# RupertLuo/Valley

Hardware: AMD Instinct MI355X
Metric: frames/sec ViT-L/14 encode + prefill tokens/sec (13B) (higher is better)
Workload: dtype bf16

## Files before the change

valley_amd/csrc/attention.hip:

```cpp
#include <cstdlib>
#include "common.hpp"
#include "../../include/valley_hip.h"

namespace {

constexpr float LOG2E = 1.4426950408889634f;
constexpr float NEG_BIG = -1.0e30f;

#ifndef VLY_DECODE_MERGE_FENCE
#define VLY_DECODE_MERGE_FENCE 0
#endif
#ifndef VLY_VIT_PRIO
#define VLY_VIT_PRIO 0
#endif
#ifndef VLY_VIT_STAGGER
#define VLY_VIT_STAGGER 0
#endif
#ifndef VLY_VIT_TIMING
#define VLY_VIT_TIMING 0
#endif
#ifndef VLY_VIT_STAGE2
#define VLY_VIT_STAGE2 1
#endif
#ifndef VLY_VIT_ROT
// ... 222 lines not shown
#pragma unroll
            for (int kk = 0; kk < 2; ++kk) {
                const bf16x8 kf = *(const bf16x8*)(sK + (t * 16 + l15) * 128 + (((kk * 4 + g) ^ (l15 & 7)) << 4));
                acc = mfma16(kf, qf[kk], acc);
            }
#if VLY_VIT_FOLD
            s[t] = acc;
#else
            s[t] = acc * sc;
#endif
            if ((t & 3) == 3) asm volatile("" ::: "memory");
        }
#if VLY_VIT_PRIO
        __builtin_amdgcn_s_setprio(0);
#endif
#pragma unroll
        for (int r = 0; r < 4; ++r)
            if (g != 0 || r != 0) s[VNT - 1][r] = NEG_BIG;
#if VLY_VIT_TIMING
        asm volatile("" : "+v"(s[VNT - 1][0]));
        VLY_VSTAMP();
#endif

        float m = NEG_BIG;
        float l = 0.f;
#if VLY_VIT_FOLD
#pragma unroll
        for (int t = 0; t < VNT; ++t) {
            m = __builtin_fmaxf(__builtin_fmaxf(m, s[t][0]), s[t][1]);
            m = __builtin_fmaxf(__builtin_fmaxf(m, s[t][2]), s[t][3]);
        }
        m = rows4_max(m);
        {
            const float nm = -m * sc;
            float l2 = 0.f;
#pragma unroll
            for (int t = 0; t < VNT; ++t) {
                const float p0 = sm_exp2(__builtin_fmaf(s[t][0], sc, nm)), p1 = sm_exp2(__builtin_fmaf(s[t][1], sc, nm));
                const float p2 = sm_exp2(__builtin_fmaf(s[t][2], sc, nm)), p3 = sm_exp2(__builtin_fmaf(s[t][3], sc, nm));
                s[t] = f32x4{p0, p1, p2, p3};
                l += p0 + p1;
                l2 += p2 + p3;
            }
            l += l2;
        }
#else
#pragma unroll
        for (int t = 0; t < VNT; ++t)
#pragma unroll
            for (int r = 0; r < 4; ++r) m = fmaxf(m, s[t][r]);
        m = rows4_max(m);
#pragma unroll
        for (int t = 0; t < VNT; ++t)
#pragma unroll
            for (int r = 0; r < 4; ++r) {
                const float p = sm_exp2(s[t][r] - m);
                s[t][r] = p;
                l += p;
            }
#endif
        l = rows4_sum(l);

#if VLY_VIT_TIMING
        asm volatile("" : "+v"(l));
        VLY_VSTAMP();
#endif
        f32x4 o[4];
#pragma unroll
        for (int dt = 0; dt < 4; ++dt) o[dt] = f32x4{0.f, 0.f, 0.f, 0.f};
#if VLY_VIT_PRIO
        __builtin_amdgcn_s_setprio(1);
#endif
#pragma unroll
        for (int c = 0; c < VNC; ++c) {
            u32x4 pk;
            pk[0] = pack_h2(s[2 * c][0], s[2 * c][1]);
            pk[1] = pack_h2(s[2 * c][2], s[2 * c][3]);
            if (2 * c + 1 < VNT) {
                pk[2] = pack_h2(s[2 * c + 1][0], s[2 * c + 1][1]);
                pk[3] = pack_h2(s[2 * c + 1][2], s[2 * c + 1][3]);
            } else {
                pk[2] = 0u;
                pk[3] = 0u;
            }
            const bf16x8 pf = __builtin_bit_cast(bf16x8, pk);
#pragma unroll
            for (int dt = 0; dt < 4; ++dt) {
                const uint16_t* vp = sVt + (dt * 16 + l15) * VT_STRIDE + 32 * c + 4 * g;
                const u32x2 lo = *(const u32x2*)vp;
                const u32x2 hi = *(const u32x2*)(vp + hi16);
                u32x4 vv;
                vv[0] = lo[0]; vv[1] = lo[1]; vv[2] = hi[0]; vv[3] = hi[1];
                o[dt] = mfma16(__builtin_bit_cast(bf16x8, vv), pf, o[dt]);
            }
            asm volatile("" ::: "memory");
        }
#if VLY_VIT_PRIO
        __builtin_amdgcn_s_setprio(0);
#endif
#if VLY_VIT_TIMING
        asm volatile("" : "+v"(o[3][3]));
        VLY_VSTAMP();
#endif
        {
            const float inv = 1.f / l;
            uint16_t* op = out + ((size_t)f * VN + min(q, VN - 1)) * 1024 + h * 64;
            {
                uint32_t y[2][4];
#pragma unroll
                for (int w = 0; w < 2; ++w) {
                    uint32_t d[4];
#pragma unroll
                    for (int dt = 0; dt < 4; ++dt) d[dt] = pack_h2(o[dt][2 * w] * inv, o[dt][2 * w + 1] * inv);
                    const auto p01 = __builtin_amdgcn_permlane16_swap(d[0], d[1], false, false);
                    const auto p23 = __builtin_amdgcn_permlane16_swap(d[2], d[3], false, false);
                    const auto q0 = __builtin_amdgcn_permlane32_swap(p01[0], p23[0], false, false);
                    const auto q1 = __builtin_amdgcn_permlane32_swap(p01[1], p23[1], false, false);
                    y[w][0] = q0[0]; y[w][1] = q1[0]; y[w][2] = q0[1]; y[w][3] = q1[1];
                }
#if VLY_VIT_STORE_LINES
                const u32x4 pa = {y[0][0], y[1][0], y[0][1], y[1][1]}, pb = {y[0][2], y[1][2], y[0][3], y[1][3]};
                u32x4 px;
#pragma unroll
                for (int i = 0; i < 4; ++i) px[i] = __builtin_amdgcn_update_dpp(0u, pb[i], 0x128, 0xf, 0xf, false);
                const bool lo8 = l15 < 8;
                const int q1 = lo8 ? q : q - 8, q2 = lo8 ? q + 8 : q;
                uint16_t* ob = out + (size_t)f * VN * 1024 + h * 64 + 16 * g;
                if (q1 < VN) *(u32x4*)(ob + (size_t)q1 * 1024 + (lo8 ? 0 : 8)) = lo8 ? pa : px;
                if (q2 < VN) *(u32x4*)(ob + (size_t)q2 * 1024 + (lo8 ? 8 : 0)) = lo8 ? px : pa;
                (void)op;
#else
                if (q < VN) {
                    u32x4* dst = (u32x4*)(op + 16 * g);
                    dst[0] = u32x4{y[0][0], y[1][0], y[0][1], y[1][1]};
                    dst[1] = u32x4{y[0][2], y[1][2], y[0][3], y[1][3]};
                }
#endif
            }
        }
        VLY_VSTAMP();
    }
#if VLY_VIT_TIMING
    if (ts_row && lane == 0 && tsn < VTS_N) ts_row[VTS_N - 1] = (unsigned long long)tsn;
#endif
}
#undef VLY_VSTAMP

typedef __attribute__((ext_vector_type(4))) short s16x4;
#include "attention_vit_persist.inc"
#include "attention_vit_pp.inc"

#ifndef VLY_LNW
#define VLY_LNW 8
#endif
constexpr int LNW = VLY_LNW;

VLY_DEVICE bf16x8 vt_frag256(const char* lo_addr) {
    typedef __attribute__((address_space(3))) s16x4 lds_s16x4;
    const s16x4 lo = __builtin_amdgcn_ds_read_tr16_b64_v4i16((lds_s16x4*)(lo_addr));
    const s16x4 hi = __builtin_amdgcn_ds_read_tr16_b64_v4i16((lds_s16x4*)(lo_addr + 16 * 256));
    return bf16x8{lo[0], lo[1], lo[2], lo[3], hi[0], hi[1], hi[2], hi[3]};
}

constexpr int L2_TILE = 64 * 256;
constexpr int L2_BUF = 2 * L2_TILE;

__global__ void __launch_bounds__(LNW * 64, 4) llama_attn2_kernel(const uint16_t* __restrict__ qkv, const uint16_t* __restrict__ kc,
                                                                 const uint16_t* __restrict__ vc, const uint8_t* __restrict__ key_valid,
                                                                 uint16_t* __restrict__ out, int S, int heads, int past,
                                                                 const int32_t* __restrict__ past_dev, int kv_stride, int ctx_max) {
    static_assert(LNW == 8, "16 + 16 pieces on 8 waves");
    __shared__ __attribute__((aligned(16))) char smem[2 * L2_BUF];
    const int tid = threadIdx.x, lane = tid & 63;
    const int wave = __builtin_amdgcn_readfirstlane(tid >> 6);
    const int l15 = lane & 15, g = lane >> 4;
    const int h = blockIdx.x, b = blockIdx.y, qb = (int)gridDim.z - 1 - (int)blockIdx.z;
    const int Hq = heads * 128;
    if (past_dev) past = min(*past_dev, ctx_max - S);
    const int kv_len = past + S;

    const int q = qb * (LNW * 16) + wave * 16 + l15;
    const int qc = min(q, S - 1);
    const int qpos = past + q;
    const int q_last = min(qb * (LNW * 16) + LNW * 16 - 1, S - 1);
    const int wave_qpos_max = past + min(qb * (LNW * 16) + wave * 16 + 15, S - 1);
    const int kv_end = min(past + q_last + 1, kv_len);
    const int ntiles = (kv_end + 63) >> 6;

    const size_t head_off = ((size_t)b * heads + h) * (size_t)ctx_max * 128;
    const __amdgpu_buffer_rsrc_t rsK = vly_rsrc(kc + head_off), rsV = vly_rsrc(vc + head_off);
    const __amdgpu_buffer_rsrc_t rsM = vly_rsrc(key_valid ? key_valid + (size_t)b * kv_stride : key_valid);
    const uint32_t lds0 = (uint32_t)(uintptr_t)(__attribute__((address_space(3))) char*)smem;
    const uint32_t hb = 0u;
    uint32_t okraw = 1u;
    bool okin = false;
    auto stage = [&](int kt, int buf) {
        const int kv0 = kt * 64;
#pragma unroll
        for (int pp = 0; pp < 2; ++pp) {
            const int pc = 2 * wave + pp, row = 4 * pc + (lane >> 4), cp = lane & 15;
            const uint32_t rb = hb + (uint32_t)min(kv0 + row, kv_len - 1) * 256u;
            const uint32_t voK = rb + (uint32_t)((cp ^ (row & 15)) << 4);
            const uint32_t voV = rb + (uint32_t)((cp ^ ((row & 7) << 1)) << 4);
            const uint32_t dst = __builtin_amdgcn_readfirstlane(lds0 + (uint32_t)buf * L2_BUF + (uint32_t)pc * 1024u);
            asm volatile("s_mov_b32 m0, %0" ::"s"(dst) : "memory");
            asm volatile("s_nop 0" ::: "memory");
            asm volatile("buffer_load_dwordx4 %0, %1, 0 offen lds" ::"v"(voK), "s"(rsK) : "memory");
            asm volatile("s_mov_b32 m0, %0" ::"s"(dst + (uint32_t)L2_TILE) : "memory");
            asm volatile("s_nop 0" ::: "memory");
            asm volatile("buffer_load_dwordx4 %0, %1, 0 offen lds" ::"v"(voV), "s"(rsV) : "memory");
        }
        const int kvl = kv0 + lane;
        okin = kvl < kv_len;
        if (key_valid) okraw = (uint32_t)__builtin_amdgcn_raw_buffer_load_b8(rsM, (uint32_t)min(kvl, kv_len - 1), 0, 0);
    };
    const int vr = 4 * g + (l15 >> 2);
    const int vbase0 = L2_TILE + vr * 256 + (l15 & 1) * 8 + (((l15 & 3) >> 1) << 4), vx0 = (vr & 7) << 5;

    if (ntiles > 0) stage(0, 0);
    const uint16_t* qp = qkv + ((size_t)b * S + qc) * 3 * Hq + h * 128;
    bf16x8 qf[4];
#pragma unroll
    for (int kk = 0; kk < 4; ++kk) qf[kk] = *(const bf16x8*)(qp + kk * 32 + g * 8);

    const float sc = 0.08838834764831845f * LOG2E;
    float m = NEG_BIG, l = 0.f;
    f32x4 o[8];
#pragma unroll
    for (int dt = 0; dt < 8; ++dt) o[dt] = f32x4{0.f, 0.f, 0.f, 0.f};

    for (int kt = 0; kt < ntiles; ++kt) {
        const int kv0 = kt * 64, buf = kt & 1;
        const char* sK = smem + buf * L2_BUF;
        __builtin_amdgcn_s_waitcnt(0x0f70);
        __syncthreads();
        const unsigned long long vmask = __ballot(okin && (okraw & 0xffu) != 0u);
        if (kt + 1 < ntiles) stage(kt + 1, buf ^ 1);
        if (kv0 > wave_qpos_max) continue;
        const int vbase = opaque_i32(vbase0), vx = opaque_i32(vx0);

        f32x4 s[4];
#pragma unroll
        for (int t = 0; t < 4; ++t) {
            f32x4 acc = {0.f, 0.f, 0.f, 0.f};
#pragma unroll
            for (int kk = 0; kk < 4; ++kk) {
                const bf16x8 kf = *(const bf16x8*)(sK + (t * 16 + l15) * 256 + (((kk * 4 + g) ^ l15) << 4));
                acc = mfma16(kf, qf[kk], acc);
            }
#pragma unroll
            for (int r = 0; r < 4; ++r) {
                const int kl = t * 16 + 4 * g + r;
                const bool vis = ((vmask >> kl) & 1ull) && (kv0 + kl <= qpos);
                s[t][r] = vis ? acc[r] * sc : NEG_BIG;
            }
        }
        float rm = NEG_BIG;
#pragma unroll
        for (int t = 0; t < 4; ++t)
#pragma unroll
            for (int r = 0; r < 4; ++r) rm = fmaxf(rm, s[t][r]);
        rm = rows4_max(rm);
        const float mn = fmaxf(m, rm);
        const float alpha = sm_exp2(m - mn);
        m = mn;
        float ps = 0.f;
#pragma unroll
        for (int t = 0; t < 4; ++t)
#pragma unroll
            for (int r = 0; r < 4; ++r) {
                const float p = sm_exp2(s[t][r] - mn);
                s[t][r] = p;
                ps += p;
            }
        l = l * alpha + ps;
#pragma unroll
        for (int dt = 0; dt < 8; ++dt) o[dt] *= alpha;
#pragma unroll
        for (int c = 0; c < 2; ++c) {
            u32x4 pk;
            pk[0] = pack_h2(s[2 * c][0], s[2 * c][1]);
            pk[1] = pack_h2(s[2 * c][2], s[2 * c][3]);
            pk[2] = pack_h2(s[2 * c + 1][0], s[2 * c + 1][1]);
            pk[3] = pack_h2(s[2 * c + 1][2], s[2 * c + 1][3]);
            const bf16x8 pf = __builtin_bit_cast(bf16x8, pk);
#pragma unroll
            for (int dt = 0; dt < 8; ++dt)
                o[dt] = mfma16(vt_frag256(sK + vbase + ((dt << 5) ^ vx) + c * 8192), pf, o[dt]);
        }
    }
    l = rows4_sum(l);
    if (q < S) {
        const float inv = 1.f / l;
        uint16_t* op = out + ((size_t)b * S + q) * Hq + h * 128 + 4 * g;
#pragma unroll
        for (int dt = 0; dt < 8; ++dt) {
            u32x2 pk;
            pk[0] = pack_h2(o[dt][0] * inv, o[dt][1] * inv);
            pk[1] = pack_h2(o[dt][2] * inv, o[dt][3] * inv);
            *(u32x2*)(op + dt * 16) = pk;
        }
    }
}

constexpr int DEC_MAX_CTX = 8192;

__global__ void __launch_bounds__(256) decode_attn_kernel(const uint16_t* __restrict__ qkv, const uint16_t* __restrict__ kc,
                                                          const uint16_t* __restrict__ vc, const uint8_t* __restrict__ key_valid,
                                                          uint16_t* __restrict__ out, int heads, int past,
                                                          const int32_t* __restrict__ past_dev, int kv_stride, int ctx_max) {
    __shared__ float sc[DEC_MAX_CTX];
    __shared__ __attribute__((aligned(16))) float qs[128];
    __shared__ float red[8];
    __shared__ __attribute__((aligned(16))) float acc_s[16][128];
    const int tid = threadIdx.x, lane = tid & 63, wave = tid >> 6;
    const int h = blockIdx.x, b = blockIdx.y;
    const int Hq = heads * 128;
    if (past_dev) past = min(*past_dev, ctx_max - 1);
    const int kv_len = past + 1;
    const uint16_t* qp = qkv + (size_t)b * 3 * Hq + h * 128;
    if (tid < 128) qs[tid] = h2f(qp[tid]) * (0.08838834764831845f * LOG2E);
    __syncthreads();
    const uint16_t* kbase = kc + ((size_t)b * heads + h) * ctx_max * 128;
    const uint16_t* vbase = vc + ((size_t)b * heads + h) * ctx_max * 128;
    const uint8_t* kvld = key_valid ? key_valid + (size_t)b * kv_stride : nullptr;

    float m = NEG_BIG;
    for (int j = tid; j < kv_len; j += 256) {
        float s = NEG_BIG;
        if (!kvld || kvld[j]) {
            const u32x4* kr = (const u32x4*)(kbase + (size_t)j * 128);
            float a = 0.f;
#pragma unroll
            for (int c = 0; c < 16; ++c) {
                const u32x4 kk = kr[c];
                const f32x4 q0 = *(const f32x4*)(qs + 8 * c), q1 = *(const f32x4*)(qs + 8 * c + 4);
                a = fmaf(h_lo(kk[0]), q0[0], a); a = fmaf(h_hi(kk[0]), q0[1], a);
                a = fmaf(h_lo(kk[1]), q0[2], a); a = fmaf(h_hi(kk[1]), q0[3], a);
                a = fmaf(h_lo(kk[2]), q1[0], a); a = fmaf(h_hi(kk[2]), q1[1], a);
                a = fmaf(h_lo(kk[3]), q1[2], a); a = fmaf(h_hi(kk[3]), q1[3], a);
            }
            s = a;
        }
        sc[j] = s;
        m = fmaxf(m, s);
    }
    m = wave_max(m);
    if (lane == 0) red[wave] = m;
    __syncthreads();
    m = fmaxf(fmaxf(red[0], red[1]), fmaxf(red[2], red[3]));
    float l = 0.f;
    for (int j = tid; j < kv_len; j += 256) {
        const float p = sm_exp2(sc[j] - m);
        sc[j] = p;
        l += p;
    }
    l = wave_sum(l);
    if (lane == 0) red[4 + wave] = l;
    __syncthreads();
    l = red[4] + red[5] + red[6] + red[7];

    const int kg = tid >> 4, dc = tid & 15;
    float o[8];
#pragma unroll
    for (int i = 0; i < 8; ++i) o[i] = 0.f;
    for (int j0 = kg; j0 < kv_len; j0 += 64) {
        u32x4 vv[4];
        float pp[4];
#pragma unroll
        for (int u = 0; u < 4; ++u) {
            const int j = j0 + 16 * u;
            const bool in = j < kv_len;
            pp[u] = in ? sc[j] : 0.f;
            vv[u] = *(const u32x4*)(vbase + (size_t)(in ? j : kg) * 128 + 8 * dc);
        }
#pragma unroll
        for (int u = 0; u < 4; ++u) {
            const float p = pp[u];
            o[0] = fmaf(p, h_lo(vv[u][0]), o[0]); o[1] = fmaf(p, h_hi(vv[u][0]), o[1]);
            o[2] = fmaf(p, h_lo(vv[u][1]), o[2]); o[3] = fmaf(p, h_hi(vv[u][1]), o[3]);
            o[4] = fmaf(p, h_lo(vv[u][2]), o[4]); o[5] = fmaf(p, h_hi(vv[u][2]), o[5]);
            o[6] = fmaf(p, h_lo(vv[u][3]), o[6]); o[7] = fmaf(p, h_hi(vv[u][3]), o[7]);
        }
    }
#pragma unroll
    for (int i = 0; i < 8; ++i) acc_s[kg][8 * dc + i] = o[i];
    __syncthreads();
    if (tid < 128) {
        float t = 0.f;
#pragma unroll
        for (int k2 = 0; k2 < 16; ++k2) t += acc_s[k2][tid];
        out[(size_t)b * Hq + h * 128 + tid] = f2h(t / l);
    }
}

__global__ void __launch_bounds__(512) decode_fused_kernel(const uint16_t* __restrict__ qkv, uint16_t* __restrict__ kc,
                                                           uint16_t* __restrict__ vc, const float* __restrict__ cos_t,
                                                           const float* __restrict__ sin_t, const uint8_t* __restrict__ key_valid,
                                                           uint16_t* __restrict__ out, int heads, int past,
                                                           const int32_t* __restrict__ past_dev, int kv_stride, int ctx_max,
                                                           int past_row_stride) {
    __shared__ float sc[512];
    __shared__ __attribute__((aligned(16))) float qs[128];
    __shared__ __attribute__((aligned(16))) float knew[128];
    __shared__ __attribute__((aligned(16))) float vnew[128];
    __shared__ float red[16];
    __shared__ __attribute__((aligned(16))) float acc_s[32][128];
    const int tid = threadIdx.x, lane = tid & 63, wave = tid >> 6;
    const int h = blockIdx.x, b = blockIdx.y;
    const int Hq = heads * 128;
    if (past_dev) past = min(past_dev[(size_t)b * past_row_stride], ctx_max - 1);
    const int pos = past, kv_len = past + 1;
    const uint16_t* qp = qkv + (size_t)b * 3 * Hq + h * 128;
    uint16_t* kbase = kc + ((size_t)b * heads + h) * ctx_max * 128;
    uint16_t* vbase = vc + ((size_t)b * heads + h) * ctx_max * 128;
    const uint8_t* kvld = key_valid ? key_valid + (size_t)b * kv_stride : nullptr;

    if (tid < 64) {
        const float cs = cos_t[(size_t)pos * 64 + tid], sn = sin_t[(size_t)pos * 64 + tid];
        const float q0 = h2f(qp[tid]), q1 = h2f(qp[tid + 64]);
        const float k0 = h2f(qp[Hq + tid]), k1 = h2f(qp[Hq + tid + 64]);
        const float scale = 0.08838834764831845f * LOG2E;
        qs[tid] = h2f(f2h(rope_rot(q0, q1, cs, sn, -1.f))) * scale;
        qs[tid + 64] = h2f(f2h(rope_rot(q1, q0, cs, sn, 1.f))) * scale;
        const uint16_t r0 = f2h(rope_rot(k0, k1, cs, sn, -1.f)), r1 = f2h(rope_rot(k1, k0, cs, sn, 1.f));
        knew[tid] = h2f(r0);
        knew[tid + 64] = h2f(r1);
        kbase[(size_t)pos * 128 + tid] = r0;
        kbase[(size_t)pos * 128 + tid + 64] = r1;
    } else if (tid < 192) {
        const int d = tid - 64;
        const uint16_t v = qp[2 * Hq + d];
        vnew[d] = h2f(v);
        vbase[(size_t)pos * 128 + d] = v;
    }
    __syncthreads();

    const int kg = tid >> 4, dc = tid & 15;
    float o[8];
#pragma unroll
    for (int i = 0; i < 8; ++i) o[i] = 0.f;
    float m_run = NEG_BIG, l_run = 0.f;

    for (int c0 = 0; c0 < kv_len; c0 += 512) {
        u32x4 vv[16];
#pragma unroll
        for (int u = 0; u < 16; ++u) {
            const int j = c0 + kg + 32 * u;
            vv[u] = (j < pos) ? *(const u32x4*)(vbase + (size_t)j * 128 + 8 * dc) : u32x4{0u, 0u, 0u, 0u};
        }
        const int jk = c0 + tid;
        float s = NEG_BIG;
        if (jk < kv_len && (!kvld || kvld[jk])) {
            float a = 0.f;
            if (jk < pos) {
                const u32x4* kr = (const u32x4*)(kbase + (size_t)jk * 128);
                u32x4 kk[16];
#pragma unroll
                for (int c = 0; c < 16; ++c) kk[c] = kr[c];
#pragma unroll
                for (int c = 0; c < 16; ++c) {
                    const f32x4 q0 = *(const f32x4*)(qs + 8 * c), q1 = *(const f32x4*)(qs + 8 * c + 4);
                    a = fmaf(h_lo(kk[c][0]), q0[0], a); a = fmaf(h_hi(kk[c][0]), q0[1], a);
                    a = fmaf(h_lo(kk[c][1]), q0[2], a); a = fmaf(h_hi(kk[c][1]), q0[3], a);
                    a = fmaf(h_lo(kk[c][2]), q1[0], a); a = fmaf(h_hi(kk[c][2]), q1[1], a);
                    a = fmaf(h_lo(kk[c][3]), q1[2], a); a = fmaf(h_hi(kk[c][3]), q1[3], a);
                }
            } else {
#pragma unroll 8
                for (int d = 0; d < 128; ++d) a = fmaf(knew[d], qs[d], a);
            }
            s = a;
        }
        float mc = wave_max(s);
        if (lane == 0) red[wave] = mc;
        __syncthreads();
        mc = red[0];
#pragma unroll
        for (int w = 1; w < 8; ++w) mc = fmaxf(mc, red[w]);
        const float m_new = fmaxf(m_run, mc);
        const float alpha = sm_exp2(m_run - m_new);
        const float p = s > 0.5f * NEG_BIG ? sm_exp2(s - m_new) : 0.f;
        sc[tid] = p;
        float lc = wave_sum(p);
        if (lane == 0) red[8 + wave] = lc;
        __syncthreads();
        lc = red[8];
#pragma unroll
        for (int w = 1; w < 8; ++w) lc += red[8 + w];
        l_run = vly_mul_add(l_run, alpha, lc);
        m_run = m_new;
#pragma unroll
        for (int i = 0; i < 8; ++i) o[i] *= alpha;
#pragma unroll
        for (int u = 0; u < 16; ++u) {
            const int jl = kg + 32 * u;
            const float pj = sc[jl];
            if (c0 + jl == pos) {
#pragma unroll
                for (int i = 0; i < 8; ++i) o[i] = fmaf(pj, vnew[8 * dc + i], o[i]);
            } else {
                o[0] = fmaf(pj, h_lo(vv[u][0]), o[0]); o[1] = fmaf(pj, h_hi(vv[u][0]), o[1]);
                o[2] = fmaf(pj, h_lo(vv[u][1]), o[2]); o[3] = fmaf(pj, h_hi(vv[u][1]), o[3]);
                o[4] = fmaf(pj, h_lo(vv[u][2]), o[4]); o[5] = fmaf(pj, h_hi(vv[u][2]), o[5]);
                o[6] = fmaf(pj, h_lo(vv[u][3]), o[6]); o[7] = fmaf(pj, h_hi(vv[u][3]), o[7]);
            }
        }
        __syncthreads();
    }
#pragma unroll
    for (int i = 0; i < 8; ++i) acc_s[kg][8 * dc + i] = o[i];
    __syncthreads();
    if (tid < 128) {
        float t = 0.f;
#pragma unroll
        for (int k2 = 0; k2 < 32; ++k2) t += acc_s[k2][tid];
        out[(size_t)b * Hq + h * 128 + tid] = f2h(t / l_run);
    }
}

VLY_DEVICE void split_publish(float* p, float v, bool write_through) {
    if (write_through) __hip_atomic_store(p, v, __ATOMIC_RELAXED, __HIP_MEMORY_SCOPE_AGENT);
    else *p = v;
}
VLY_DEVICE void split_merge_if_last(const float* __restrict__ partials, uint16_t* __restrict__ merged, unsigned* __restrict__ arrivals,
                                    int heads, int h, int b, float* flag_lds) {
    asm volatile("s_waitcnt vmcnt(0)" ::: "memory");
    __syncthreads();
    unsigned* ctr = arrivals + (size_t)b * heads + h;
    if (threadIdx.x == 0) {
#if VLY_DECODE_MERGE_FENCE
        __builtin_amdgcn_fence(__ATOMIC_RELEASE, "agent");
        asm volatile("s_waitcnt vmcnt(0)" ::: "memory");
#endif
        const unsigned t = __hip_atomic_fetch_add(ctr, 1u, __ATOMIC_RELAXED, __HIP_MEMORY_SCOPE_AGENT);
        flag_lds[0] = t == VLY_DECODE_SPLITS - 1 ? 1.f : 0.f;
        if (t == VLY_DECODE_SPLITS - 1) {
            __hip_atomic_store(ctr, 0u, __ATOMIC_RELAXED, __HIP_MEMORY_SCOPE_AGENT);
#if VLY_DECODE_MERGE_FENCE
            __builtin_amdgcn_fence(__ATOMIC_ACQUIRE, "agent");
#endif
        }
    }
    __syncthreads();
    if (flag_lds[0] == 0.f || threadIdx.x >= 32) return;
    const float* hb = partials + ((size_t)b * heads + h) * (VLY_DECODE_SPLITS * 132);
    float ms[VLY_DECODE_SPLITS], ls[VLY_DECODE_SPLITS];
    float os[VLY_DECODE_SPLITS][4];
#pragma unroll
    for (int sp = 0; sp < VLY_DECODE_SPLITS; ++sp) {
        ms[sp] = __hip_atomic_load(hb + sp * 132, __ATOMIC_RELAXED, __HIP_MEMORY_SCOPE_AGENT);
        ls[sp] = __hip_atomic_load(hb + sp * 132 + 1, __ATOMIC_RELAXED, __HIP_MEMORY_SCOPE_AGENT);
#pragma unroll
        for (int r = 0; r < 4; ++r)
            os[sp][r] = __hip_atomic_load(hb + sp * 132 + 4 + 4 * (int)threadIdx.x + r, __ATOMIC_RELAXED, __HIP_MEMORY_SCOPE_AGENT);
    }
    float mx = ms[0];
#pragma unroll
    for (int sp = 1; sp < VLY_DECODE_SPLITS; ++sp) mx = fmaxf(mx, ms[sp]);
    float L = 0.f, O[4] = {0.f, 0.f, 0.f, 0.f};
#pragma unroll
    for (int sp = 0; sp < VLY_DECODE_SPLITS; ++sp) {
        const float w = exp2f(ms[sp] - mx);
        L = fmaf(ls[sp], w, L);
#pragma unroll
        for (int r = 0; r < 4; ++r) O[r] = fmaf(os[sp][r], w, O[r]);
    }
    u32x2 pk;
    pk[0] = pack_h2(O[0] / L, O[1] / L);
    pk[1] = pack_h2(O[2] / L, O[3] / L);
    *(u32x2*)(merged + ((size_t)b * heads + h) * 128 + 4 * threadIdx.x) = pk;
}

__global__ void __launch_bounds__(256) decode_split_kernel(const uint16_t* __restrict__ qkv, uint16_t* __restrict__ kc,
                                                           uint16_t* __restrict__ vc, const float* __restrict__ cos_t,
                                                           const float* __restrict__ sin_t, const uint8_t* __restrict__ key_valid,
                                                           float* __restrict__ partials, int heads, int past,
                                                           const int32_t* __restrict__ past_dev, int kv_stride, int ctx_max,
                                                           int past_row_stride, uint16_t* __restrict__ merged,
                                                           unsigned* __restrict__ arrivals) {
    __shared__ float sc[256];
    __shared__ __attribute__((aligned(16))) float qs[128];
    __shared__ __attribute__((aligned(16))) float knew[128];
    __shared__ __attribute__((aligned(16))) float vnew[128];
    __shared__ float red[8];
    __shared__ __attribute__((aligned(16))) float acc_s[16][128];
    const int tid = threadIdx.x, lane = tid & 63, wave = tid >> 6;
    const bool spread = gridDim.z != VLY_DECODE_SPLITS;
    const int h = spread ? blockIdx.y : blockIdx.x, b = spread ? blockIdx.z : blockIdx.y, sp = spread ? blockIdx.x : blockIdx.z;
    const int Hq = heads * 128;
    if (past_dev) past = min(past_dev[(size_t)b * past_row_stride], ctx_max - 1);
    const int pos = past, kv_len = past + 1;
    const int chunk = (((kv_len + VLY_DECODE_SPLITS - 1) / VLY_DECODE_SPLITS) + 63) & ~63;
    const int lo = sp * chunk, hi = min(lo + chunk, kv_len);
    const bool owner = pos >= lo && pos < hi;
    const uint16_t* qp = qkv + (size_t)b * 3 * Hq + h * 128;
    uint16_t* kbase = kc + ((size_t)b * heads + h) * ctx_max * 128;
    uint16_t* vbase = vc + ((size_t)b * heads + h) * ctx_max * 128;
    const uint8_t* kvld = key_valid ? key_valid + (size_t)b * kv_stride : nullptr;
    float* part = partials + (((size_t)b * heads + h) * VLY_DECODE_SPLITS + sp) * 132;
    if (lo >= hi) {
        if (tid < 132) split_publish(part + tid, tid == 0 ? NEG_BIG : 0.f, merged != nullptr);
        if (merged) split_merge_if_last(partials, merged, arrivals, heads, h, b, sc);
        return;
    }
    const int t63 = tid & 63;
    const float cs = cos_t[(size_t)pos * 64 + t63], sn = sin_t[(size_t)pos * 64 + t63];
    const uint16_t q0r = qp[t63], q1r = qp[t63 + 64], k0r = qp[Hq + t63], k1r = qp[Hq + t63 + 64], vr = qp[2 * Hq + ((tid - 64) & 127)];
    u32x4 vv[16], kk[16];
    uint8_t kvalid = 1;
    const int jmax = max(min(hi, pos) - 1, 0);
    auto request = [&](int c0) {
        if (c0 + (tid & ~63) < hi) {
            const u32x4* kr = (const u32x4*)(kbase + (size_t)min(c0 + tid, jmax) * 128);
#pragma unroll
            for (int c = 0; c < 16; ++c) kk[c] = kr[c];
        }
        if (kvld) kvalid = kvld[min(c0 + tid, hi - 1)];
#pragma unroll
        for (int u = 0; u < 8; ++u) vv[u] = *(const u32x4*)(vbase + (size_t)min(c0 + (tid >> 4) + 16 * u, jmax) * 128 + 8 * (tid & 15));
        if (hi - c0 > 128) {
#pragma unroll
            for (int u = 8; u < 16; ++u) vv[u] = *(const u32x4*)(vbase + (size_t)min(c0 + (tid >> 4) + 16 * u, jmax) * 128 + 8 * (tid & 15));
        } else {
#pragma unroll
            for (int u = 8; u < 16; ++u) vv[u] = u32x4{0u, 0u, 0u, 0u};
        }
    };
    request(lo);
    if (tid < 64) {
        const float q0 = h2f(q0r), q1 = h2f(q1r);
        const float scale = 0.08838834764831845f * LOG2E;
        qs[tid] = h2f(f2h(rope_rot(q0, q1, cs, sn, -1.f))) * scale;
        qs[tid + 64] = h2f(f2h(rope_rot(q1, q0, cs, sn, 1.f))) * scale;
        if (owner) {
            const float k0 = h2f(k0r), k1 = h2f(k1r);
            const uint16_t r0 = f2h(rope_rot(k0, k1, cs, sn, -1.f)), r1 = f2h(rope_rot(k1, k0, cs, sn, 1.f));
            knew[tid] = h2f(r0);
            knew[tid + 64] = h2f(r1);
            kbase[(size_t)pos * 128 + tid] = r0;
            kbase[(size_t)pos * 128 + tid + 64] = r1;
        }
    } else if (tid < 192 && owner) {
        const int d = tid - 64;
        vnew[d] = h2f(vr);
        vbase[(size_t)pos * 128 + d] = vr;
    }
    __syncthreads();

    const int kg = tid >> 4, dc = tid & 15;
    float o[8];
#pragma unroll
    for (int i = 0; i < 8; ++i) o[i] = 0.f;
    float m_run = NEG_BIG, l_run = 0.f;
#pragma unroll 1
    for (int c0 = lo; c0 < hi; c0 += 256) {
        if (c0 != lo) request(c0);
#pragma unroll
        for (int u = 0; u < 16; ++u) {
            const int j = c0 + kg + 16 * u;
            if (!(j < hi && j < pos)) vv[u] = u32x4{0u, 0u, 0u, 0u};
        }
        const int jk = c0 + tid;
        float s = NEG_BIG;
        if (jk < hi && kvalid) {
            float a = 0.f;
            if (jk < pos) {
#pragma unroll
                for (int c = 0; c < 16; ++c) {
                    const f32x4 q0 = *(const f32x4*)(qs + 8 * c), q1 = *(const f32x4*)(qs + 8 * c + 4);
                    a = fmaf(h_lo(kk[c][0]), q0[0], a); a = fmaf(h_hi(kk[c][0]), q0[1], a);
                    a = fmaf(h_lo(kk[c][1]), q0[2], a); a = fmaf(h_hi(kk[c][1]), q0[3], a);
                    a = fmaf(h_lo(kk[c][2]), q1[0], a); a = fmaf(h_hi(kk[c][2]), q1[1], a);
                    a = fmaf(h_lo(kk[c][3]), q1[2], a); a = fmaf(h_hi(kk[c][3]), q1[3], a);
                }
            } else {
#pragma unroll 8
                for (int d = 0; d < 128; ++d) a = fmaf(knew[d], qs[d], a);
            }
            s = a;
        }
        float mc = wave_max(s);
        if (lane == 0) red[wave] = mc;
        __syncthreads();
        mc = fmaxf(fmaxf(red[0], red[1]), fmaxf(red[2], red[3]));
        const float m_new = fmaxf(m_run, mc);
        const float alpha = sm_exp2(m_run - m_new);
        const float p = s > 0.5f * NEG_BIG ? sm_exp2(s - m_new) : 0.f;
        sc[tid] = p;
        float lc = wave_sum(p);
        if (lane == 0) red[4 + wave] = lc;
        __syncthreads();
        lc = red[4] + red[5] + red[6] + red[7];
        l_run = vly_mul_add(l_run, alpha, lc);
        m_run = m_new;
#pragma unroll
        for (int i = 0; i < 8; ++i) o[i] *= alpha;
#pragma unroll
        for (int u = 0; u < 16; ++u) {
            const int jl = kg + 16 * u;
            const float pj = sc[jl];
            if (owner && c0 + jl == pos) {
#pragma unroll
                for (int i = 0; i < 8; ++i) o[i] = fmaf(pj, vnew[8 * dc + i], o[i]);
            } else {
                o[0] = fmaf(pj, h_lo(vv[u][0]), o[0]); o[1] = fmaf(pj, h_hi(vv[u][0]), o[1]);
                o[2] = fmaf(pj, h_lo(vv[u][1]), o[2]); o[3] = fmaf(pj, h_hi(vv[u][1]), o[3]);
                o[4] = fmaf(pj, h_lo(vv[u][2]), o[4]); o[5] = fmaf(pj, h_hi(vv[u][2]), o[5]);
                o[6] = fmaf(pj, h_lo(vv[u][3]), o[6]); o[7] = fmaf(pj, h_hi(vv[u][3]), o[7]);
            }
        }
        __syncthreads();
    }
#pragma unroll
    for (int i = 0; i < 8; ++i) acc_s[kg][8 * dc + i] = o[i];
    __syncthreads();
    if (tid < 128) {
        float t = 0.f;
#pragma unroll
        for (int k2 = 0; k2 < 16; ++k2) t += acc_s[k2][tid];
        split_publish(part + 4 + tid, t, merged != nullptr);
    } else if (tid < 132) {
        split_publish(part + tid - 128, tid == 128 ? m_run : tid == 129 ? l_run : 0.f, merged != nullptr);
    }
    if (merged) split_merge_if_last(partials, merged, arrivals, heads, h, b, sc);
}


template <typename T> VLY_DEVICE float probs_ld(const T* p);
template <> VLY_DEVICE float probs_ld<uint16_t>(const uint16_t* p) { return h2f(*p); }
template <> VLY_DEVICE float probs_ld<float>(const float* p) { return *p; }

template <typename T>
__global__ void __launch_bounds__(256) attn_probs_kernel(const T* __restrict__ qkv, const T* __restrict__ kc,
                                                         const uint8_t* __restrict__ key_valid, float* __restrict__ out, int S,
                                                         int heads, int past, int kv_stride, int ctx_max) {
    extern __shared__ float pr_sc[];
    __shared__ float qs[128];
    __shared__ float red[8];
    const int tid = threadIdx.x, lane = tid & 63, wave = tid >> 6;
    const int i = blockIdx.x, h = blockIdx.y, b = blockIdx.z;
    const int kv_len = past + S, vis = past + i + 1, Hq = heads * 128;
    const T* q = qkv + ((size_t)b * S + i) * 3 * Hq + h * 128;
    const T* kb = kc + ((size_t)b * heads + h) * ctx_max * 128;
    const uint8_t* kvld = key_valid ? key_valid + (size_t)b * kv_stride : nullptr;
    if (tid < 128) qs[tid] = probs_ld(q + tid) * (0.08838834764831845f * LOG2E);
    __syncthreads();
    float m = NEG_BIG;
    for (int j = tid; j < kv_len; j += 256) {
        float s = NEG_BIG;
        if (j < vis && (!kvld || kvld[j])) {
            const T* kr = kb + (size_t)j * 128;
            float a = 0.f;
#pragma unroll 8
            for (int d = 0; d < 128; ++d) a = fmaf(probs_ld(kr + d), qs[d], a);
            s = a;
        }
        pr_sc[j] = s;
        m = fmaxf(m, s);
    }
    m = wave_max(m);
    if (lane == 0) red[wave] = m;
    __syncthreads();
    m = fmaxf(fmaxf(red[0], red[1]), fmaxf(red[2], red[3]));
    float l = 0.f;
    for (int j = tid; j < kv_len; j += 256) {
        const float s = pr_sc[j];
        const float p = s > 0.5f * NEG_BIG ? sm_exp2(s - m) : 0.f;
        pr_sc[j] = p;
        l += p;
    }
    l = wave_sum(l);
    if (lane == 0) red[4 + wave] = l;
    __syncthreads();
    l = red[4] + red[5] + red[6] + red[7];
    const float inv = l > 0.f ? 1.f / l : 0.f;
    float* o = out + (((size_t)b * heads + h) * S + i) * kv_len;
    for (int j = tid; j < kv_len; j += 256) o[j] = pr_sc[j] * inv;
}

#ifndef VLY_EXPERIMENTAL
#define VLY_EXPERIMENTAL 0
#endif
#if VLY_EXPERIMENTAL
#include "attention_ab.inc"
#endif

}

#if VLY_VIT_TIMING
extern "C" int vlydbg_vit_timing_read(unsigned long long* host) { return (int)hipMemcpyFromSymbol(host, HIP_SYMBOL(vit_ts), sizeof(unsigned long long) * VTS_WG * VNW * VTS_N); }
#endif

#ifndef VLY_VIT_PERSIST_MIN
#define VLY_VIT_PERSIST_MIN 1
#endif
#ifndef VLY_VIT_PP
#define VLY_VIT_PP 0
#endif
constexpr int VIT_PERSIST_MIN_FRAMES = VLY_VIT_PERSIST_MIN;
extern "C" int vly_vit_attention(const void* qkv, void* out, int F, void* stream) {
    if (F <= 0 || ((uintptr_t)qkv & 15) || ((uintptr_t)out & 15)) { vly_set_error("vly_vit_attention: bad args F=%d (qkv and out 16-byte aligned)", F); return -22; }
    const char* sel = getenv("VLY_VIT_ATTN");
    const int ver = sel ? atoi(sel) : 0;
    if (ver == 4 || ver == 5 || (ver != 1 && F >= VIT_PERSIST_MIN_FRAMES)) {
        static const int cus = [] {
            int dev = 0, n = 0;
            (void)hipGetDevice(&dev);
            (void)hipDeviceGetAttribute(&n, hipDeviceAttributeMultiprocessorCount, dev);
            return n > 0 ? n : 256;
        }();
        const int nheads = F * 16;
        if ((size_t)F * VN * VLD * 2 >= ((size_t)1 << 32)) { vly_set_error("vly_vit_attention: F=%d exceeds the 4 GB buffer descriptor", F); return -22; }
        if (ver == 5 || VLY_VIT_PP) {
            hipLaunchKernelGGL(vit_attn_pp_kernel, dim3(nheads < 2 * cus ? nheads : 2 * cus), dim3(PPW * 64), 0, (hipStream_t)stream,
                               (const uint16_t*)qkv, (uint16_t*)out, nheads);
            return vly_check_launch("vly_vit_attention");
        }
        hipLaunchKernelGGL(vit_attn_persist_kernel, dim3(nheads < cus ? nheads : cus), dim3(VPW * 64), 0, (hipStream_t)stream,
                           (const uint16_t*)qkv, (uint16_t*)out, nheads);
        return vly_check_launch("vly_vit_attention");
    }
    hipLaunchKernelGGL(vit_attn_kernel, dim3(F * 16), dim3(VNW * 64), 0, (hipStream_t)stream, (const uint16_t*)qkv, (uint16_t*)out);
    return vly_check_launch("vly_vit_attention");
}

extern "C" int vly_llama_attention(const void* qkv, const void* kcache, const void* vcache, const uint8_t* key_valid,
                                   int key_valid_stride, void* out, int B, int S, int heads, int past_len,
                                   const int32_t* past_len_dev, int ctx_max, void* stream) {
    if (B <= 0 || S <= 0 || heads <= 0 || past_len < 0 || past_len + S > ctx_max || B > 65535 || heads > 65535 ||
        ((uintptr_t)qkv & 15) || ((uintptr_t)kcache & 15) || ((uintptr_t)vcache & 15) || ((uintptr_t)out & 7)) {
        vly_set_error("vly_llama_attention: bad args B=%d S=%d heads=%d past=%d ctx_max=%d", B, S, heads, past_len, ctx_max);
        return -22;
    }
    if (key_valid && key_valid_stride < past_len + S) {
        vly_set_error("vly_llama_attention: key_valid_stride %d < kv_len %d", key_valid_stride, past_len + S);
        return -22;
    }
    if (S == 1 && ctx_max <= DEC_MAX_CTX) {
        hipLaunchKernelGGL(decode_attn_kernel, dim3(heads, B), dim3(256), 0, (hipStream_t)stream, (const uint16_t*)qkv,
                           (const uint16_t*)kcache, (const uint16_t*)vcache, key_valid, (uint16_t*)out, heads, past_len,
                           past_len_dev, key_valid_stride, ctx_max);
        return vly_check_launch("vly_llama_attention(decode)");
    }
#if VLY_EXPERIMENTAL
    static const int ver = getenv("VLY_LLAMA_ATTN") ? atoi(getenv("VLY_LLAMA_ATTN")) : 2;
#else
    constexpr int ver = 2;
#endif
    if ((size_t)ctx_max * 256 >= ((size_t)1 << 32)) {
        vly_set_error("vly_llama_attention: ctx_max %d exceeds the 4 GB a (batch, head) cache row may span", ctx_max);
        return -22;
    }
    if (ver == 2) {
        hipLaunchKernelGGL(llama_attn2_kernel, dim3(heads, B, (S + 16 * LNW - 1) / (16 * LNW)), dim3(LNW * 64), 0, (hipStream_t)stream,
                           (const uint16_t*)qkv, (const uint16_t*)kcache, (const uint16_t*)vcache, key_valid, (uint16_t*)out,
                           S, heads, past_len, past_len_dev, key_valid_stride, ctx_max);
        return vly_check_launch("vly_llama_attention");
    }
#if VLY_EXPERIMENTAL
    hipLaunchKernelGGL(llama_attn_kernel, dim3(heads, B, (S + 16 * LNW - 1) / (16 * LNW)), dim3(LNW * 64), 0, (hipStream_t)stream,
                       (const uint16_t*)qkv, (const uint16_t*)kcache, (const uint16_t*)vcache, key_valid, (uint16_t*)out,
                       S, heads, past_len, past_len_dev, key_valid_stride, ctx_max);
    return vly_check_launch("vly_llama_attention");
#else
    return -22;
#endif
}

extern "C" int vly_decode_attention(const void* qkv, void* kcache, void* vcache, const float* cos_table, const float* sin_table,
                                    const uint8_t* key_valid, int key_valid_stride, void* out, int B, int heads, int past_len,
                                    const int32_t* past_len_dev, int ctx_max, void* stream) {
    if (B <= 0 || heads <= 0 || past_len < 0 || past_len + 1 > ctx_max || B > 65535 || heads > 65535 ||
        ((uintptr_t)qkv & 15) || ((uintptr_t)kcache & 15) || ((uintptr_t)vcache & 15) || ((uintptr_t)out & 7) || !cos_table || !sin_table) {
        vly_set_error("vly_decode_attention: bad args B=%d heads=%d past=%d ctx_max=%d", B, heads, past_len, ctx_max);
        return -22;
    }
    if (key_valid && key_valid_stride < past_len + 1) {
        vly_set_error("vly_decode_attention: key_valid_stride %d < kv_len %d", key_valid_stride, past_len + 1);
        return -22;
    }
    hipLaunchKernelGGL(decode_fused_kernel, dim3(heads, B), dim3(512), 0, (hipStream_t)stream, (const uint16_t*)qkv,
                       (uint16_t*)kcache, (uint16_t*)vcache, cos_table, sin_table, key_valid, (uint16_t*)out, heads, past_len,
                       past_len_dev, key_valid_stride, ctx_max, 0);
    return vly_check_launch("vly_decode_attention");
}

extern "C" int vly_decode_attention_rows(const void* qkv, void* kcache, void* vcache, const float* cos_table, const float* sin_table,
                                         const uint8_t* key_valid, int key_valid_stride, void* out, int B, int heads,
                                         const int32_t* past_len_rows, int ctx_max, void* stream) {
    if (B <= 0 || heads <= 0 || !past_len_rows || B > 65535 || heads > 65535 || ((uintptr_t)qkv & 15) || ((uintptr_t)kcache & 15) ||
        ((uintptr_t)vcache & 15) || ((uintptr_t)out & 7) || !cos_table || !sin_table || (key_valid && key_valid_stride < ctx_max)) {
        vly_set_error("vly_decode_attention_rows: bad args B=%d heads=%d ctx_max=%d key_valid_stride=%d", B, heads, ctx_max, key_valid_stride);
        return -22;
    }
    hipLaunchKernelGGL(decode_fused_kernel, dim3(heads, B), dim3(512), 0, (hipStream_t)stream, (const uint16_t*)qkv,
                       (uint16_t*)kcache, (uint16_t*)vcache, cos_table, sin_table, key_valid, (uint16_t*)out, heads, 0,
                       past_len_rows, key_valid_stride, ctx_max, 1);
    return vly_check_launch("vly_decode_attention_rows");
}

static int decode_split_launch(const char* name, const void* qkv, void* kcache, void* vcache, const float* cos_table,
                               const float* sin_table, const uint8_t* key_valid, int key_valid_stride, float* partials, int B,
                               int heads, int past_len, const int32_t* past_len_dev, int past_len_dev_stride, int ctx_max,
                               void* merged, unsigned* arrivals, void* stream);

#if VLY_EXPERIMENTAL
extern "C" int vly_decode_attention_split(const void* qkv, void* kcache, void* vcache, const float* cos_table, const float* sin_table,
                                          const uint8_t* key_valid, int key_valid_stride, float* partials, int B, int heads,
                                          int past_len, const int32_t* past_len_dev, int past_len_dev_stride, int ctx_max,
                                          void* stream) {
    return decode_split_launch("vly_decode_attention_split", qkv, kcache, vcache, cos_table, sin_table, key_valid, key_valid_stride,
                               partials, B, heads, past_len, past_len_dev, past_len_dev_stride, ctx_max, nullptr, nullptr, stream);
}
#endif

extern "C" int vly_decode_attention_merged(const void* qkv, void* kcache, void* vcache, const float* cos_table, const float* sin_table,
                                           const uint8_t* key_valid, int key_valid_stride, float* partials, void* out,
                                           uint32_t* arrivals, int B, int heads, int past_len, const int32_t* past_len_dev,
                                           int past_len_dev_stride, int ctx_max, void* stream) {
    if (!out || ((uintptr_t)out & 7) || !arrivals || ((uintptr_t)arrivals & 3)) {
        vly_set_error("vly_decode_attention_merged: out (8-byte aligned) and arrivals (B * heads zeroed uint32) are required");
        return -22;
    }
    return decode_split_launch("vly_decode_attention_merged", qkv, kcache, vcache, cos_table, sin_table, key_valid, key_valid_stride,
                               partials, B, heads, past_len, past_len_dev, past_len_dev_stride, ctx_max, out, arrivals, stream);
}

static int decode_split_launch(const char* name, const void* qkv, void* kcache, void* vcache, const float* cos_table,
                               const float* sin_table, const uint8_t* key_valid, int key_valid_stride, float* partials, int B,
                               int heads, int past_len, const int32_t* past_len_dev, int past_len_dev_stride, int ctx_max,
                               void* merged, unsigned* arrivals, void* stream) {
    if (B <= 0 || heads <= 0 || past_len < 0 || past_len + 1 > ctx_max || B > 65535 || heads > 65535 || ((uintptr_t)qkv & 15) ||
        ((uintptr_t)kcache & 15) || ((uintptr_t)vcache & 15) || !partials || ((uintptr_t)partials & 15) || !cos_table || !sin_table ||
        past_len_dev_stride < 0 || past_len_dev_stride > 1 || (past_len_dev_stride == 1 && !past_len_dev)) {
        vly_set_error("%s: bad args B=%d heads=%d past=%d ctx_max=%d", name, B, heads, past_len, ctx_max);
        return -22;
    }
    if (key_valid && key_valid_stride < (past_len_dev ? ctx_max : past_len + 1)) {
        vly_set_error("%s: key_valid_stride %d too short", name, key_valid_stride);
        return -22;
    }
    static const bool spread = getenv("VLY_DECODE_SPLIT_SPREAD") && atoi(getenv("VLY_DECODE_SPLIT_SPREAD")) != 0 && VLY_DECODE_SPLITS != 1;
    const dim3 grid = spread && B != VLY_DECODE_SPLITS ? dim3(VLY_DECODE_SPLITS, heads, B) : dim3(heads, B, VLY_DECODE_SPLITS);
    hipLaunchKernelGGL(decode_split_kernel, grid, dim3(256), 0, (hipStream_t)stream, (const uint16_t*)qkv,
                       (uint16_t*)kcache, (uint16_t*)vcache, cos_table, sin_table, key_valid, partials, heads, past_len, past_len_dev,
                       key_valid_stride, ctx_max, past_len_dev_stride, (uint16_t*)merged, arrivals);
    return vly_check_launch(name);
}

extern "C" int vly_llama_attention_probs(const void* qkv, const void* kcache, const uint8_t* key_valid, int key_valid_stride,
                                         float* out, int B, int S, int heads, int past_len, int ctx_max, int inputs_f32,
                                         void* stream) {
    const int kv_len = past_len + S;
    if (B <= 0 || S <= 0 || heads <= 0 || past_len < 0 || kv_len > ctx_max || kv_len > 16000 || B > 65535 || heads > 65535 || !qkv ||
        !kcache || !out) {
        vly_set_error("vly_llama_attention_probs: bad args B=%d S=%d heads=%d past=%d ctx_max=%d (kv_len <= 16000)", B, S, heads,
                      past_len, ctx_max);
        return -22;
    }
    if (key_valid && key_valid_stride < kv_len) {
        vly_set_error("vly_llama_attention_probs: key_valid_stride %d < kv_len %d", key_valid_stride, kv_len);
        return -22;
    }
    const dim3 grid(S, heads, B), block(256);
    const size_t lds = (size_t)kv_len * 4;
    if (inputs_f32)
        hipLaunchKernelGGL(attn_probs_kernel<float>, grid, block, lds, (hipStream_t)stream, (const float*)qkv, (const float*)kcache,
                           key_valid, out, S, heads, past_len, key_valid_stride, ctx_max);
    else
        hipLaunchKernelGGL(attn_probs_kernel<uint16_t>, grid, block, lds, (hipStream_t)stream, (const uint16_t*)qkv,
                           (const uint16_t*)kcache, key_valid, out, S, heads, past_len, key_valid_stride, ctx_max);
    return vly_check_launch("vly_llama_attention_probs");
}
```

Before: 1747.

## Add llama prefill attention kernel with 32 query rows per wave

New measurement: 1750 (median of 6 runs). Within noise of the previous version (+0.2%).

```diff
diff --git a/valley_amd/csrc/attention.hip b/valley_amd/csrc/attention.hip
--- a/valley_amd/csrc/attention.hip
+++ b/valley_amd/csrc/attention.hip
@@ -548,6 +548,265 @@
         }
     }
 }
+
+#ifndef VLY_L3NW
+#define VLY_L3NW 4
+#endif
+#ifndef VLY_LLAMA3_MIN_S
+#define VLY_LLAMA3_MIN_S 64
+#endif
+#ifndef VLY_L3_TIMING
+#define VLY_L3_TIMING 0
+#endif
+constexpr int L3NW = VLY_L3NW;
+constexpr int L3Q = 32 * L3NW;
+
+#if VLY_L3_TIMING
+constexpr int L3TS_WG = 1024, L3TS_N = 40;
+__device__ unsigned long long l3_ts[L3TS_WG * L3NW * L3TS_N];
+#define VLY_L3STAMP()                                                                                    \
+    do {                                                                                                  \
+        if (ts_row && lane == 0 && tsn < L3TS_N - 1) ts_row[tsn] = __builtin_readcyclecounter();           \
+        ++tsn;                                                                                            \
+    } while (0)
+#else
+#define VLY_L3STAMP() do {} while (0)
+#endif
+
+VLY_DEVICE void store_row128(uint16_t* row_ptr, const f32x4 (&o)[8], float inv, int g, bool live) {
+#pragma unroll
+    for (int hh = 0; hh < 2; ++hh) {
+        uint32_t y[2][4];
+#pragma unroll
+        for (int w = 0; w < 2; ++w) {
+            uint32_t d[4];
+#pragma unroll
+            for (int dt = 0; dt < 4; ++dt) d[dt] = pack_h2(o[4 * hh + dt][2 * w] * inv, o[4 * hh + dt][2 * w + 1] * inv);
+            const auto p01 = __builtin_amdgcn_permlane16_swap(d[0], d[1], false, false);
+            const auto p23 = __builtin_amdgcn_permlane16_swap(d[2], d[3], false, false);
+            const auto q0 = __builtin_amdgcn_permlane32_swap(p01[0], p23[0], false, false);
+            const auto q1 = __builtin_amdgcn_permlane32_swap(p01[1], p23[1], false, false);
+            y[w][0] = q0[0]; y[w][1] = q1[0]; y[w][2] = q0[1]; y[w][3] = q1[1];
+        }
+        if (live) {
+            u32x4* dst = (u32x4*)(row_ptr + 64 * hh + 16 * g);
+            dst[0] = u32x4{y[0][0], y[1][0], y[0][1], y[1][1]};
+            dst[1] = u32x4{y[0][2], y[1][2], y[0][3], y[1][3]};
+        }
+    }
+}
+
+template <bool B> struct l3_bool { static constexpr bool value = B; };
+
+__global__ void __launch_bounds__(L3NW * 64, 2) llama_attn3_kernel(const uint16_t* __restrict__ qkv, const uint16_t* __restrict__ kc,
+                                                                  const uint16_t* __restrict__ vc, const uint8_t* __restrict__ key_valid,
+                                                                  uint16_t* __restrict__ out, int S, int heads, int past,
+                                                                  const int32_t* __restrict__ past_dev, int kv_stride, int ctx_max) {
+    static_assert(L3NW == 8 || L3NW == 4, "16 + 16 pieces on 8 or 4 waves");
+    constexpr int PPW = 16 / L3NW;
+    __shared__ __attribute__((aligned(16))) char smem[2 * L2_BUF];
+    const int tid = threadIdx.x, lane = tid & 63;
+    const int wave = __builtin_amdgcn_readfirstlane(tid >> 6);
+    const int l15 = lane & 15, g = lane >> 4;
+    const int h = blockIdx.x, b = blockIdx.y, qb = (int)gridDim.z - 1 - (int)blockIdx.z;
+    const int Hq = heads * 128;
+    if (past_dev) past = min(*past_dev, ctx_max - S);
+    const int kv_len = past + S;
+#if VLY_L3_TIMING
+    const unsigned wg_lin = (blockIdx.z * gridDim.y + blockIdx.y) * gridDim.x + blockIdx.x;
+    unsigned long long* ts_row = wg_lin < (unsigned)L3TS_WG ? l3_ts + ((size_t)wg_lin * L3NW + wave) * L3TS_N : nullptr;
+    int tsn = 0;
+    VLY_L3STAMP();
+    if (ts_row && lane == 0) {
+        unsigned xcc;
+        asm volatile("s_getreg_b32 %0, hwreg(HW_REG_XCC_ID)" : "=s"(xcc));
+        ts_row[tsn] = (unsigned long long)(xcc & 0xf);
+    }
+    ++tsn;
+#endif
+
+    const int qw = qb * L3Q + wave * 32;
+    int qpos[2], set_qpos_max[2];
+#pragma unroll
+    for (int cs = 0; cs < 2; ++cs) {
+        qpos[cs] = past + qw + 16 * cs + l15;
+        set_qpos_max[cs] = past + min(qw + 16 * cs + 15, S - 1);
+    }
+    const int q_last = min(qb * L3Q + L3Q - 1, S - 1);
+    const int kv_end = min(past + q_last + 1, kv_len);
+    const int ntiles = (kv_end + 63) >> 6;
+
+    const size_t head_off = ((size_t)b * heads + h) * (size_t)ctx_max * 128;
+    const __amdgpu_buffer_rsrc_t rsK = vly_rsrc(kc + head_off), rsV = vly_rsrc(vc + head_off);
+    const __amdgpu_buffer_rsrc_t rsM = vly_rsrc(key_valid ? key_valid + (size_t)b * kv_stride : key_valid);
+    const uint32_t lds0 = (uint32_t)(uintptr_t)(__attribute__((address_space(3))) char*)smem;
+    uint32_t okraw = 1u;
+    bool okin = false;
+    auto stage = [&](int kt, int buf) {
+        const int kv0 = kt * 64;
+#pragma unroll
+        for (int pp = 0; pp < PPW; ++pp) {
+            const int pc = PPW * wave + pp, row = 4 * pc + (lane >> 4), cp = lane & 15;
+            const uint32_t rb = (uint32_t)min(kv0 + row, kv_len - 1) * 256u;
+            const uint32_t voK = rb + (uint32_t)((cp ^ (row & 15)) << 4);
+            const uint32_t voV = rb + (uint32_t)((cp ^ ((row & 7) << 1)) << 4);
+            const uint32_t dst = __builtin_amdgcn_readfirstlane(lds0 + (uint32_t)buf * L2_BUF + (uint32_t)pc * 1024u);
+            asm volatile("s_mov_b32 m0, %0" ::"s"(dst) : "memory");
+            asm volatile("s_nop 0" ::: "memory");
+            asm volatile("buffer_load_dwordx4 %0, %1, 0 offen lds" ::"v"(voK), "s"(rsK) : "memory");
+            asm volatile("s_mov_b32 m0, %0" ::"s"(dst + (uint32_t)L2_TILE) : "memory");
+            asm volatile("s_nop 0" ::: "memory");
+            asm volatile("buffer_load_dwordx4 %0, %1, 0 offen lds" ::"v"(voV), "s"(rsV) : "memory");
+        }
+        const int kvl = kv0 + lane;
+        okin = kvl < kv_len;
+        if (key_valid) okraw = (uint32_t)__builtin_amdgcn_raw_buffer_load_b8(rsM, (uint32_t)min(kvl, kv_len - 1), 0, 0);
+    };
+    const int vr = 4 * g + (l15 >> 2);
+    const int vbase0 = L2_TILE + vr * 256 + (l15 & 1) * 8 + (((l15 & 3) >> 1) << 4), vx0 = (vr & 7) << 5;
+
+    if (ntiles > 0) stage(0, 0);
+    bf16x8 qf[2][4];
+#pragma unroll
+    for (int cs = 0; cs < 2; ++cs) {
+        const uint16_t* qp = qkv + ((size_t)b * S + min(qw + 16 * cs + l15, S - 1)) * 3 * Hq + h * 128;
+#pragma unroll
+        for (int kk = 0; kk < 4; ++kk) qf[cs][kk] = *(const bf16x8*)(qp + kk * 32 + g * 8);
+    }
+
+    const float sc = 0.08838834764831845f * LOG2E;
+    float m[2] = {NEG_BIG, NEG_BIG}, l[2] = {0.f, 0.f};
+    f32x4 o[2][8];
+#pragma unroll
+    for (int cs = 0; cs < 2; ++cs)
+#pragma unroll
+        for (int dt = 0; dt < 8; ++dt) o[cs][dt] = f32x4{0.f, 0.f, 0.f, 0.f};
+
+    auto tile_begin = [&](int kt) {
+        __builtin_amdgcn_s_waitcnt(0x0f70);
+        __syncthreads();
+        VLY_L3STAMP();
+        const unsigned long long vmask = __ballot(okin && (okraw & 0xffu) != 0u);
+        if (kt + 1 < ntiles) stage(kt + 1, (kt & 1) ^ 1);
+        return vmask;
+    };
+    auto tile = [&](auto both_c, int kt, unsigned long long vmask) {
+        constexpr int CS0 = decltype(both_c)::value ? 0 : 1;
+        const int kv0 = kt * 64;
+        const char* sK = smem + (kt & 1) * L2_BUF;
+        const int vbase = opaque_i32(vbase0), vx = opaque_i32(vx0);
+        {
+            unsigned long long vism[2];
+#pragma unroll
+            for (int cs = CS0; cs < 2; ++cs) {
+                const int lim = qpos[cs] - kv0 - 4 * g;
+                const unsigned long long cm = lim < 0 ? 0ull : (lim >= 63 ? ~0ull : ((2ull << lim) - 1ull));
+                vism[cs] = (vmask >> (4 * g)) & cm;
+            }
+            f32x4 s[2][4];
+#pragma unroll
+            for (int t = 0; t < 4; ++t) {
+                f32x4 acc[2] = {{0.f, 0.f, 0.f, 0.f}, {0.f, 0.f, 0.f, 0.f}};
+#pragma unroll
+                for (int kk = 0; kk < 4; ++kk) {
+                    const bf16x8 kf = *(const bf16x8*)(sK + (t * 16 + l15) * 256 + (((kk * 4 + g) ^ l15) << 4));
+#pragma unroll
+                    for (int cs = CS0; cs < 2; ++cs) acc[cs] = mfma16(kf, qf[cs][kk], acc[cs]);
+                }
+#pragma unroll
+                for (int cs = CS0; cs < 2; ++cs) s[cs][t] = acc[cs];
+            }
+            constexpr unsigned long long USED = 0x000f000f000f000full;
+            bool whole = true;
+#pragma unroll
+            for (int cs = CS0; cs < 2; ++cs) whole = whole && (vism[cs] & USED) == USED;
+            if (__all(whole)) {
+#pragma unroll
+                for (int cs = CS0; cs < 2; ++cs)
+#pragma unroll
+                    for (int t = 0; t < 4; ++t)
+#pragma unroll
+                        for (int r = 0; r < 4; ++r) s[cs][t][r] = s[cs][t][r] * sc;
+            } else {
+#pragma unroll
+                for (int cs = CS0; cs < 2; ++cs)
+#pragma unroll
+                    for (int t = 0; t < 4; ++t)
+#pragma unroll
+                        for (int r = 0; r < 4; ++r) {
+                            const bool vis = (vism[cs] >> (t * 16 + r)) & 1ull;
+                            s[cs][t][r] = vis ? s[cs][t][r] * sc : NEG_BIG;
+                        }
+            }
+            VLY_L3STAMP();
+#pragma unroll
+            for (int cs = CS0; cs < 2; ++cs) {
+                float rm = NEG_BIG;
+#pragma unroll
+                for (int t = 0; t < 4; ++t)
+#pragma unroll
+                    for (int r = 0; r < 4; ++r) rm = fmaxf(rm, s[cs][t][r]);
+                rm = rows4_max(rm);
+                const float mn = fmaxf(m[cs], rm);
+                const float alpha = sm_exp2(m[cs] - mn);
+                m[cs] = mn;
+                float ps = 0.f;
+#pragma unroll
+                for (int t = 0; t < 4; ++t)
+#pragma unroll
+                    for (int r = 0; r < 4; ++r) {
+                        const float p = sm_exp2(s[cs][t][r] - mn);
+                        s[cs][t][r] = p;
+                        ps += p;
+                    }
+                l[cs] = l[cs] * alpha + ps;
+#pragma unroll
+                for (int dt = 0; dt < 8; ++dt) o[cs][dt] *= alpha;
+            }
+            VLY_L3STAMP();
+#pragma unroll
+            for (int c = 0; c < 2; ++c) {
+                bf16x8 pf[2];
+#pragma unroll
+                for (int cs = CS0; cs < 2; ++cs) {
+                    u32x4 pk;
+                    pk[0] = pack_h2(s[cs][2 * c][0], s[cs][2 * c][1]);
+                    pk[1] = pack_h2(s[cs][2 * c][2], s[cs][2 * c][3]);
+                    pk[2] = pack_h2(s[cs][2 * c + 1][0], s[cs][2 * c + 1][1]);
+                    pk[3] = pack_h2(s[cs][2 * c + 1][2], s[cs][2 * c + 1][3]);
+                    pf[cs] = __builtin_bit_cast(bf16x8, pk);
+                }
+#pragma unroll
+                for (int dt = 0; dt < 8; ++dt) {
+                    const bf16x8 vf = vt_frag256(sK + vbase + ((dt << 5) ^ vx) + c * 8192);
+#pragma unroll
+                    for (int cs = CS0; cs < 2; ++cs) o[cs][dt] = mfma16(vf, pf[cs], o[cs][dt]);
+                }
+            }
+            VLY_L3STAMP();
+        }
+    };
+    const bool dead = qw >= S;
+    const int n0 = dead ? 0 : min(ntiles, (set_qpos_max[0] >> 6) + 1), n1 = dead ? 0 : min(ntiles, (set_qpos_max[1] >> 6) + 1);
+    int kt = 0;
+    for (; kt < n0; ++kt) tile(l3_bool<true>{}, kt, tile_begin(kt));
+    for (; kt < n1; ++kt) tile(l3_bool<false>{}, kt, tile_begin(kt));
+    for (; kt < ntiles; ++kt) {
+        (void)tile_begin(kt);
+        VLY_L3STAMP(); VLY_L3STAMP(); VLY_L3STAMP();
+    }
+#pragma unroll
+    for (int cs = 0; cs < 2; ++cs) {
+        const float lt = rows4_sum(l[cs]);
+        const int q = qw + 16 * cs + l15;
+        store_row128(out + ((size_t)b * S + min(q, S - 1)) * Hq + h * 128, o[cs], 1.f / lt, g, q < S);
+    }
+#if VLY_L3_TIMING
+    VLY_L3STAMP();
+    if (ts_row && lane == 0) ts_row[L3TS_N - 1] = (unsigned long long)tsn;
+#endif
+}
+#undef VLY_L3STAMP
 
 constexpr int DEC_MAX_CTX = 8192;
 
@@ -1034,6 +1293,9 @@
 
 }
 
+#if VLY_L3_TIMING
+extern "C" int vlydbg_l3_timing_read(unsigned long long* host) { return (int)hipMemcpyFromSymbol(host, HIP_SYMBOL(l3_ts), sizeof(unsigned long long) * L3TS_WG * L3NW * L3TS_N); }
+#endif
 #if VLY_VIT_TIMING
 extern "C" int vlydbg_vit_timing_read(unsigned long long* host) { return (int)hipMemcpyFromSymbol(host, HIP_SYMBOL(vit_ts), sizeof(unsigned long long) * VTS_WG * VNW * VTS_N); }
 #endif
@@ -1090,15 +1352,21 @@
         return vly_check_launch("vly_llama_attention(decode)");
     }
 #if VLY_EXPERIMENTAL
-    static const int ver = getenv("VLY_LLAMA_ATTN") ? atoi(getenv("VLY_LLAMA_ATTN")) : 2;
+    static const int ver = getenv("VLY_LLAMA_ATTN") ? atoi(getenv("VLY_LLAMA_ATTN")) : 3;
 #else
-    constexpr int ver = 2;
+    constexpr int ver = 3;
 #endif
     if ((size_t)ctx_max * 256 >= ((size_t)1 << 32)) {
         vly_set_error("vly_llama_attention: ctx_max %d exceeds the 4 GB a (batch, head) cache row may span", ctx_max);
         return -22;
     }
-    if (ver == 2) {
+    if (ver == 3 && S >= VLY_LLAMA3_MIN_S && !((uintptr_t)out & 15)) {
+        hipLaunchKernelGGL(llama_attn3_kernel, dim3(heads, B, (S + L3Q - 1) / L3Q), dim3(L3NW * 64), 0, (hipStream_t)stream,
+                           (const uint16_t*)qkv, (const uint16_t*)kcache, (const uint16_t*)vcache, key_valid, (uint16_t*)out,
+                           S, heads, past_len, past_len_dev, key_valid_stride, ctx_max);
+        return vly_check_launch("vly_llama_attention");
+    }
+    if (ver == 2 || ver == 3) {
         hipLaunchKernelGGL(llama_attn2_kernel, dim3(heads, B, (S + 16 * LNW - 1) / (16 * LNW)), dim3(LNW * 64), 0, (hipStream_t)stream,
                            (const uint16_t*)qkv, (const uint16_t*)kcache, (const uint16_t*)vcache, key_valid, (uint16_t*)out,
                            S, heads, past_len, past_len_dev, key_valid_stride, ctx_max);
```
